# david-jk/BigGAN-Tensorflow

Measured on AMD Instinct MI355X. Metric: BigGAN-128 train-step images/sec, higher is better.
Workload: dtype bf16; 1 GPU; BigGAN-128 ch=96 bf16 (BASELINE config 3: global batch 256, 32/GPU over 8 GPUs); img_size=128, ch=96, per_gpu_batch=256, global_batch=256, da_policy=full, g_regularization=ortho_cosine, n_labels=0, gan_type=hinge, hip_graph=False, precision=bf16, parallelism=dp1

## Files before the change

### biggan-tensorflow_amd/csrc/elementwise.hip

```cpp
#include <stdlib.h>
#include <mutex>
#include "common.h"

namespace bg {

#define EW_BLOCK 256
#define EW_MAX_BLOCKS 2048

static inline int ew_grid(int64_t work_items) {
    int64_t b = (work_items + EW_BLOCK - 1) / EW_BLOCK;
    if (b > EW_MAX_BLOCKS) b = EW_MAX_BLOCKS;
    if (b < 1) b = 1;
    return (int)b;
}

__device__ __forceinline__ float4 ldg4(const float* p) { return *reinterpret_cast<const float4*>(p); }
__device__ __forceinline__ void stg4(float* p, const float4& v) { *reinterpret_cast<float4*>(p) = v; }

template <int NQ, int VEC, class Fn, class OutT>
__global__ __launch_bounds__(EW_BLOCK) void colreduce_kernel(Fn fn, OutT* out, float* part, int64_t qstride,
                                                             int64_t rows_per_seg, int C, int rows_per_block) {
    __shared__ float red[NQ * EW_BLOCK * VEC];
    const int CV = C / VEC;
    const int tx = CV < EW_BLOCK ? CV : EW_BLOCK;
    const int lanes = EW_BLOCK / tx;
    const int cq = threadIdx.x % tx, rl = threadIdx.x / tx;
    const int seg = blockIdx.y;
    const int64_t r0 = (int64_t)blockIdx.x * rows_per_block;
    int64_t r1 = r0 + rows_per_block;
    if (r1 > rows_per_seg) r1 = rows_per_seg;
    for (int cbase = 0; cbase < CV; cbase += tx) {
        const int cv = cbase + cq;
        float acc[NQ][VEC];
#pragma unroll
        for (int q = 0; q < NQ; ++q)
#pragma unroll
            for (int j = 0; j < VEC; ++j) acc[q][j] = 0.f;
        if (cv < CV && rl < lanes) {
            float acc4[4][NQ][VEC];
#pragma unroll
            for (int u = 0; u < 4; ++u)
#pragma unroll
                for (int q = 0; q < NQ; ++q)
#pragma unroll
                    for (int j = 0; j < VEC; ++j) acc4[u][q][j] = 0.f;
            int64_t r = r0 + rl;
            for (; r + 3 * (int64_t)lanes < r1; r += 4 * (int64_t)lanes) {
#pragma unroll
                for (int u = 0; u < 4; ++u) fn(seg, r + u * (int64_t)lanes, cv * VEC, acc4[u]);
            }
            for (; r < r1; r += lanes) fn(seg, r, cv * VEC, acc4[0]);
#pragma unroll
            for (int q = 0; q < NQ; ++q)
#pragma unroll
                for (int j = 0; j < VEC; ++j)
                    acc[q][j] = (acc4[0][q][j] + acc4[1][q][j]) + (acc4[2][q][j] + acc4[3][q][j]);
        }
#pragma unroll
        for (int q = 0; q < NQ; ++q)
#pragma unroll
            for (int j = 0; j < VEC; ++j) red[(q * VEC + j) * EW_BLOCK + threadIdx.x] = acc[q][j];
        __syncthreads();
        if (rl == 0 && cv < CV) {
#pragma unroll
            for (int q = 0; q < NQ; ++q)
#pragma unroll
                for (int j = 0; j < VEC; ++j) {
                    float s = 0.f;
                    for (int l = 0; l < lanes; ++l) s += red[(q * VEC + j) * EW_BLOCK + l * tx + cq];
// ... 81 lines not shown
        return nullptr;
    }
    if (ws[dev] && !captured[dev]) {
        (void)hipDeviceSynchronize();
        (void)hipFree(ws[dev]);
    }
    ws[dev] = p;
    cap[dev] = want;
    captured[dev] = false;
    return p;
}

static bool block_partials(int grid, int C, hipStream_t s, float** part) {
    *part = grid > 1 ? colreduce_workspace((size_t)grid * C, s) : nullptr;
    return grid <= 1 || *part;
}

static void finalize_block_partials(const float* part, float* out, int grid, int C, hipStream_t s) {
    if (part)
        hipLaunchKernelGGL((colreduce_finalize_kernel<1, float>), crf_grid(C), dim3(EW_BLOCK), 0, s, part, out,
                           (int64_t)0, 1, C, grid);
}

template <int NQ, bool WIDE = false, class Fn, class OutT>
static void launch_colreduce(Fn fn, OutT* out, int64_t qstride, int64_t rows_per_seg, int nseg, int C,
                             hipStream_t s) {
    static const int env_blocks = getenv("BG_COLRED_BLOCKS") ? atoi(getenv("BG_COLRED_BLOCKS")) : 0;
    const int64_t bytes = rows_per_seg * (int64_t)nseg * C * 4;
    const int target_blocks = env_blocks > 0 ? env_blocks : (bytes > (100ll << 20) ? 192 : 128);
    int64_t blocks_per_seg = (target_blocks + nseg - 1) / nseg;
    int64_t rpb = (rows_per_seg + blocks_per_seg - 1) / blocks_per_seg;
    if (rpb < 32) rpb = 32;
    blocks_per_seg = (rows_per_seg + rpb - 1) / rpb;
    float* part = nullptr;
    if (blocks_per_seg > 1) {
        part = colreduce_workspace((size_t)blocks_per_seg * nseg * NQ * C, s);
        if (!part) {
            g_ws_error = true;
            return;
        }
    }
    dim3 grid((unsigned)blocks_per_seg, (unsigned)nseg);
    bool launched = false;
    if constexpr (WIDE) {
        if (C % 8 == 0 && rows_per_seg * (int64_t)nseg * C >= (int64_t(16) << 20)) {
            hipLaunchKernelGGL((colreduce_kernel<NQ, 8, Fn, OutT>), grid, dim3(EW_BLOCK), 0, s, fn, out, part, qstride,
                               rows_per_seg, C, (int)rpb);
            launched = true;
        }
    }
    if (!launched) {
        if (C % 4 == 0)
            hipLaunchKernelGGL((colreduce_kernel<NQ, 4, Fn, OutT>), grid, dim3(EW_BLOCK), 0, s, fn, out, part, qstride,
                               rows_per_seg, C, (int)rpb);
        else
            hipLaunchKernelGGL((colreduce_kernel<NQ, 1, Fn, OutT>), grid, dim3(EW_BLOCK), 0, s, fn, out, part, qstride,
                               rows_per_seg, C, (int)rpb);
    }
    if (part) {
        const int64_t total = (int64_t)nseg * NQ * C;
        hipLaunchKernelGGL((colreduce_finalize_kernel<NQ, OutT>), crf_grid(total), dim3(EW_BLOCK), 0, s, part, out,
                           qstride, nseg, C, (int)blocks_per_seg);
    }
}

template <int VEC>
__device__ __forceinline__ void loadv(const float* p, float (&v)[VEC]) {
    if constexpr (VEC == 4) {
        float4 t = ldg4(p);
        v[0] = t.x;
        v[1] = t.y;
        v[2] = t.z;
        v[VEC - 1] = t.w;
    } else if constexpr (VEC == 8) {
        const float4 a = ldg4(p), b = ldg4(p + 4);
        v[0] = a.x; v[1] = a.y; v[2] = a.z; v[3] = a.w;
        v[4] = b.x; v[5] = b.y; v[6] = b.z; v[VEC - 1] = b.w;
    } else {
#pragma unroll
        for (int j = 0; j < VEC; ++j) v[j] = p[j];
    }
// ... 26 lines not shown
}
template <int VEC>
__device__ __forceinline__ void storev(float* p, const float (&v)[VEC]) {
    if constexpr (VEC == 4)
        stg4(p, make_float4(v[0], v[1], v[2], v[VEC - 1]));
    else {
#pragma unroll
        for (int j = 0; j < VEC; ++j) p[j] = v[j];
    }
}
template <int VEC>
__device__ __forceinline__ void storev(__bf16* p, const float (&v)[VEC]) {
    if constexpr (VEC == 4) {
        uint2 r;
        r.x = bf16_pack2(v[0], v[1]);
        r.y = bf16_pack2(v[2], v[VEC - 1]);
        *reinterpret_cast<uint2*>(p) = r;
    } else {
#pragma unroll
        for (int j = 0; j < VEC; ++j) p[j] = (__bf16)v[j];
    }
}

template <class TX>
struct BnStatsFnT {
    const TX* x;
    int C;
    template <int VEC>
    __device__ __forceinline__ void operator()(int, int64_t r, int c, float (&acc)[2][VEC]) const {
        float v[VEC];
        loadv<VEC>(x + r * C + c, v);
#pragma unroll
        for (int j = 0; j < VEC; ++j) {
            acc[0][j] += v[j];
            acc[1][j] += v[j] * v[j];
        }
    }
};

__global__ void bn_population_kernel(const float* __restrict__ pop_mean, const float* __restrict__ pop_var, float eps,
                                     float* __restrict__ mean, float* __restrict__ rstd, int C) {
    const int c = blockIdx.x * blockDim.x + threadIdx.x;
    if (c >= C) return;
    mean[c] = pop_mean[c];
    rstd[c] = rsqrtf(pop_var[c] + eps);
}

__global__ void bn_finalize_kernel(const double* sums, double count, float eps, float momentum, int unbiased,
                                   float* mean, float* rstd, float* mm, float* mv, int C) {
    const int c = blockIdx.x * blockDim.x + threadIdx.x;
// ... 165 lines not shown
    const float *mean, *rstd, *gamma, *beta, *alpha;
    int per_sample, HW, C;
    template <int VEC>
    __device__ __forceinline__ void operator()(int n, int64_t r, int c, float (&acc)[3][VEC]) const {
        const int64_t off = ((int64_t)n * HW + r) * C + c;
        float xv[VEC], dv[VEC], mu[VEC], rs[VEC], ga[VEC], be[VEC], al[VEC];
        loadv<VEC>(x + off, xv);
        loadv<VEC>(dy + off, dv);
        loadv<VEC>(mean + c, mu);
        loadv<VEC>(rstd + c, rs);
        loadv<VEC>(gamma + (per_sample ? (int64_t)n * C : 0) + c, ga);
        loadv<VEC>(beta + (per_sample ? (int64_t)n * C : 0) + c, be);
        if (alpha) loadv<VEC>(alpha + c, al);
#pragma unroll
        for (int j = 0; j < VEC; ++j) {
            const float xh = (xv[j] - mu[j]) * rs[j];
            const float pre = xh * ga[j] + be[j];
            const float g = alpha ? dv[j] * prelu_d(pre, al[j]) : dv[j];
            acc[0][j] += g;
            acc[1][j] += g * xh;
            acc[2][j] += alpha ? dv[j] * fminf(pre, 0.f) : 0.f;
        }
    }
};

template <int VEC, class TX, class TY>
__global__ __launch_bounds__(EW_BLOCK) void bn_apply_act_bwd_dx_t_kernel(
    const TX* __restrict__ x, const TY* __restrict__ dy, const float* __restrict__ mean,
    const float* __restrict__ rstd, const float* __restrict__ gamma, const float* __restrict__ beta, int per_sample,
    const float* __restrict__ alpha, const float* __restrict__ cm, TX* dx, const TX* add, int N, int HW, int C) {
    const int CV = C / VEC;
    const int64_t total = (int64_t)N * HW * CV;
    for (int64_t i = (int64_t)blockIdx.x * EW_BLOCK + threadIdx.x; i < total; i += (int64_t)gridDim.x * EW_BLOCK) {
        const int c = (int)(i % CV) * VEC;
        const int n = (int)(i / ((int64_t)HW * CV));
        float xv[VEC], dv[VEC], mu[VEC], rs[VEC], ga[VEC], be[VEC], al[VEC], m1[VEC], m2[VEC], out[VEC];
        loadv<VEC>(x + i * VEC, xv);
        loadv<VEC>(dy + i * VEC, dv);
        loadv<VEC>(mean + c, mu);
        loadv<VEC>(rstd + c, rs);
        loadv<VEC>(gamma + (per_sample ? (int64_t)n * C : 0) + c, ga);
        loadv<VEC>(beta + (per_sample ? (int64_t)n * C : 0) + c, be);
        loadv<VEC>(cm + c, m1);
        loadv<VEC>(cm + C + c, m2);
        if (alpha) loadv<VEC>(alpha + c, al);
#pragma unroll
// ... 49 lines not shown
                    dbeta[(int64_t)n * C + c] = a[u];
                    dgamma[(int64_t)n * C + c] = b[u];
                }
            }
        }
    }
    red[0][ry][cx] = s0; red[1][ry][cx] = s1; red[2][ry][cx] = s2; red[3][ry][cx] = g0; red[4][ry][cx] = g1;
    __syncthreads();
    if (ry != 0 || !live) return;
    s0 = (red[0][0][cx] + red[0][1][cx]) + (red[0][2][cx] + red[0][3][cx]);
    s1 = (red[1][0][cx] + red[1][1][cx]) + (red[1][2][cx] + red[1][3][cx]);
    s2 = (red[2][0][cx] + red[2][1][cx]) + (red[2][2][cx] + red[2][3][cx]);
    g0 = (red[3][0][cx] + red[3][1][cx]) + (red[3][2][cx] + red[3][3][cx]);
    g1 = (red[4][0][cx] + red[4][1][cx]) + (red[4][2][cx] + red[4][3][cx]);
    if (!per_sample) {
        dbeta[c] = (float)s0;
        dgamma[c] = (float)s1;
    }
    if (dalpha) dalpha[c] = (float)s2;
    cm[c] = (float)(g0 / count);
    cm[C + c] = (float)(g1 / count);
}

__device__ __forceinline__ void bf16x8_load(const __bf16* p, float (&v)[8]) {
    const uint4 r = *reinterpret_cast<const uint4*>(p);
    v[0] = __builtin_bit_cast(float, r.x << 16); v[1] = __builtin_bit_cast(float, r.x & 0xffff0000u);
    v[2] = __builtin_bit_cast(float, r.y << 16); v[3] = __builtin_bit_cast(float, r.y & 0xffff0000u);
    v[4] = __builtin_bit_cast(float, r.z << 16); v[5] = __builtin_bit_cast(float, r.z & 0xffff0000u);
    v[6] = __builtin_bit_cast(float, r.w << 16); v[7] = __builtin_bit_cast(float, r.w & 0xffff0000u);
}
__device__ __forceinline__ void bf16x8_store(__bf16* p, const float (&v)[8]) {
    uint4 r;
    r.x = bf16_pack2(v[0], v[1]); r.y = bf16_pack2(v[2], v[3]); r.z = bf16_pack2(v[4], v[5]); r.w = bf16_pack2(v[6], v[7]);
    *reinterpret_cast<uint4*>(p) = r;
}
__device__ __forceinline__ void f32x8_load(const float* p, float (&v)[8]) {
    const float4 a = ldg4(p), b = ldg4(p + 4);
    v[0] = a.x; v[1] = a.y; v[2] = a.z; v[3] = a.w; v[4] = b.x; v[5] = b.y; v[6] = b.z; v[7] = b.w;
}

__global__ __launch_bounds__(EW_BLOCK) void bn_apply_act_fwd_bf16x8_kernel(
    const __bf16* __restrict__ x, const float* __restrict__ mean, const float* __restrict__ rstd,
    const float* __restrict__ gamma, const float* __restrict__ beta, int per_sample, const float* __restrict__ alpha,
    __bf16* __restrict__ y, int rows, int HW, int CV) {
    const int gtid = blockIdx.x * EW_BLOCK + threadIdx.x;
    const int cv = gtid % CV, c = cv * 8, C = CV * 8;
    const int rstep = (gridDim.x * EW_BLOCK) / CV;
    float mu[8], rs[8], al[8], inv[8], sh[8];
    f32x8_load(mean + c, mu);
    f32x8_load(rstd + c, rs);
    if (alpha) f32x8_load(alpha + c, al);
    int r_end = 0;
    for (int r = gtid / CV; r < rows; r += rstep) {
        if (r >= r_end) {
            const int n = per_sample ? r / HW : 0;
            r_end = per_sample ? (n + 1) * HW : rows;
            float ga[8], be[8];
            f32x8_load(gamma + (int64_t)n * C * per_sample + c, ga);
            f32x8_load(beta + (int64_t)n * C * per_sample + c, be);
#pragma unroll
            for (int j = 0; j < 8; ++j) {
                inv[j] = rs[j] * ga[j];
                sh[j] = be[j] - mu[j] * inv[j];
            }
        }
        float xv[8], out[8];
        bf16x8_load(x + (int64_t)r * C + c, xv);
#pragma unroll
        for (int j = 0; j < 8; ++j) {
            const float v = xv[j] * inv[j] + sh[j];
            out[j] = alpha ? prelu_f(v, al[j]) : v;
        }
        bf16x8_store(y + (int64_t)r * C + c, out);
    }
}

__global__ __launch_bounds__(EW_BLOCK) void bn_apply_act_bwd_dx_bf16x8_kernel(
    const __bf16* __restrict__ x, const __bf16* __restrict__ dy, const float* __restrict__ mean,
    const float* __restrict__ rstd, const float* __restrict__ gamma, const float* __restrict__ beta, int per_sample,
    const float* __restrict__ alpha, const float* __restrict__ cm, __bf16* dx, const __bf16* add, int rows, int HW,
    int CV) {
    const int gtid = blockIdx.x * EW_BLOCK + threadIdx.x;
    const int cv = gtid % CV, c = cv * 8, C = CV * 8;
    const int rstep = (gridDim.x * EW_BLOCK) / CV;
    float mu[8], rs[8], al[8], m1[8], m2[8], ga[8], be[8];
    f32x8_load(mean + c, mu);
    f32x8_load(rstd + c, rs);
    f32x8_load(cm + c, m1);
    f32x8_load(cm + C + c, m2);
    if (alpha) f32x8_load(alpha + c, al);
    int r_end = 0;
    for (int r = gtid / CV; r < rows; r += rstep) {
        if (r >= r_end) {
            const int n = per_sample ? r / HW : 0;
            r_end = per_sample ? (n + 1) * HW : rows;
            f32x8_load(gamma + (int64_t)n * C * per_sample + c, ga);
            f32x8_load(beta + (int64_t)n * C * per_sample + c, be);
        }
        float xv[8], dv[8], out[8];
        bf16x8_load(x + (int64_t)r * C + c, xv);
        bf16x8_load(dy + (int64_t)r * C + c, dv);
#pragma unroll
        for (int j = 0; j < 8; ++j) {
            const float xh = (xv[j] - mu[j]) * rs[j];
            const float pre = xh * ga[j] + be[j];
            const float g = alpha ? dv[j] * prelu_d(pre, al[j]) : dv[j];
            out[j] = rs[j] * (g * ga[j] - m1[j] - xh * m2[j]);
        }
        if (add) {
            float av[8];
            bf16x8_load(add + (int64_t)r * C + c, av);
#pragma unroll
            for (int j = 0; j < 8; ++j) out[j] += av[j];
        }
        bf16x8_store(dx + (int64_t)r * C + c, out);
    }
}

template <bool BWD>
__global__ __launch_bounds__(EW_BLOCK) void prelu_bf16x8_kernel(const __bf16* __restrict__ x, const __bf16* __restrict__ dy,
                                                                 const float* __restrict__ alpha, __bf16* out,
                                                                 const __bf16* add, int rows, int CV) {
    const int gtid = blockIdx.x * EW_BLOCK + threadIdx.x;
    const int c = (gtid % CV) * 8, C = CV * 8;
    const int rstep = (gridDim.x * EW_BLOCK) / CV;
    float al[8];
    f32x8_load(alpha + c, al);
    for (int r = gtid / CV; r < rows; r += rstep) {
        float xv[8], dv[8], o[8];
        bf16x8_load(x + (int64_t)r * C + c, xv);
        if (BWD) bf16x8_load(dy + (int64_t)r * C + c, dv);
#pragma unroll
        for (int j = 0; j < 8; ++j) o[j] = BWD ? dv[j] * prelu_d(xv[j], al[j]) : prelu_f(xv[j], al[j]);
        if (BWD && add) {
            float av[8];
            bf16x8_load(add + (int64_t)r * C + c, av);
#pragma unroll
            for (int j = 0; j < 8; ++j) o[j] += av[j];
        }
        bf16x8_store(out + (int64_t)r * C + c, o);
    }
}

__global__ __launch_bounds__(EW_BLOCK) void lincomb_bf16x8_kernel(const __bf16* __restrict__ a, const float* sa_dev, float sa,
                                                                   const __bf16* __restrict__ b, float sb,
                                                                   __bf16* __restrict__ y, int64_t n8) {
    const float s = sa_dev ? *sa_dev : sa;
    for (int64_t i = (int64_t)blockIdx.x * EW_BLOCK + threadIdx.x; i < n8; i += (int64_t)gridDim.x * EW_BLOCK) {
        float av[8], bv[8], o[8];
        bf16x8_load(a + i * 8, av);
        if (b) {
            bf16x8_load(b + i * 8, bv);
#pragma unroll
            for (int j = 0; j < 8; ++j) o[j] = s * av[j] + sb * bv[j];
        } else {
#pragma unroll
            for (int j = 0; j < 8; ++j) o[j] = s * av[j];
        }
        bf16x8_store(y + i * 8, o);
    }
}

static inline int bn_x8_grid(int64_t rows, int CV) {
    int a = CV, b = EW_BLOCK;
    while (b) { const int t = a % b; a = b; b = t; }
    const int unit = CV / a;
    int64_t want = (rows * CV + EW_BLOCK - 1) / EW_BLOCK;
    if (want > 4096) want = 4096;
    if (want < 1) want = 1;
    return (int)((want + unit - 1) / unit * unit);
}

template <int VEC, class TX, class TY>
__global__ __launch_bounds__(EW_BLOCK) void prelu_fwd_t_kernel(const TX* __restrict__ x, const float* __restrict__ alpha,
                                                                TY* __restrict__ y, int64_t total_v, int C) {
    const int CV = C / VEC;
    for (int64_t i = (int64_t)blockIdx.x * EW_BLOCK + threadIdx.x; i < total_v; i += (int64_t)gridDim.x * EW_BLOCK) {
        const int c = (int)(i % CV) * VEC;
        float xv[VEC], al[VEC], out[VEC];
        loadv<VEC>(x + i * VEC, xv);
        loadv<VEC>(alpha + c, al);
#pragma unroll
        for (int j = 0; j < VEC; ++j) out[j] = prelu_f(xv[j], al[j]);
        storev<VEC>(y + i * VEC, out);
// ... 16 lines not shown
        if (add) {
            float av[VEC];
            loadv<VEC>(add + i * VEC, av);
#pragma unroll
            for (int j = 0; j < VEC; ++j) out[j] += av[j];
        }
        storev<VEC>(dx + i * VEC, out);
    }
}

template <class TX, class TY>
struct PreluDalphaFnT {
    const TX* x;
    const TY* dy;
    int C;
    template <int VEC>
    __device__ __forceinline__ void operator()(int, int64_t r, int c, float (&acc)[1][VEC]) const {
        float xv[VEC], dv[VEC];
        loadv<VEC>(x + r * C + c, xv);
        loadv<VEC>(dy + r * C + c, dv);
#pragma unroll
        for (int j = 0; j < VEC; ++j) acc[0][j] += dv[j] * fminf(xv[j], 0.f);
    }
};

template <class T>
struct BiasGradFnT {
    const T* dy;
    int C;
    template <int VEC>
    __device__ __forceinline__ void operator()(int, int64_t r, int c, float (&acc)[1][VEC]) const {
        float dv[VEC];
        loadv<VEC>(dy + r * C + c, dv);
#pragma unroll
        for (int j = 0; j < VEC; ++j) acc[0][j] += dv[j];
    }
};

__global__ __launch_bounds__(EW_BLOCK) void prelu_dalpha_thin_kernel(float* part, const float* __restrict__ x, const float* __restrict__ dy,
                                                                     float* __restrict__ dalpha, int64_t rows, int C) {
    __shared__ float red[4][EW_BLOCK];
    float acc[4] = {0.f, 0.f, 0.f, 0.f};
    const int64_t stride = (int64_t)gridDim.x * EW_BLOCK;
    int64_t r = (int64_t)blockIdx.x * EW_BLOCK + threadIdx.x;
    for (; r + 3 * stride < rows; r += 4 * stride) {
        float xv[4][4], gv[4][4];
#pragma unroll
        for (int u = 0; u < 4; ++u)
#pragma unroll
            for (int c = 0; c < 4; ++c)
                if (c < C) {
                    xv[u][c] = x[(r + u * stride) * C + c];
                    gv[u][c] = dy[(r + u * stride) * C + c];
                }
#pragma unroll
        for (int u = 0; u < 4; ++u)
// ... 1483 lines not shown
    const int tiles = taps * ((rows_per_tap + 63) / 64) * ((cols + 63) / 64);
    hipLaunchKernelGGL(weight_pack_kernel, dim3(tiles < 2048 ? tiles : 2048), dim3(EW_BLOCK), 0, as_stream(stream), w,
                       (__bf16*)pack_p, (__bf16*)pack_t, taps, rows_per_tap, cols);
    BG_LAUNCH_CHECK();
    return BG_OK;
}

int bg_bn_stats_t(const void* x, int x_dtype, double* sums, int64_t rows, int C, void* stream) {
    BG_REQUIRE(x && sums && rows > 0 && C > 0 && BG_DT_OK(x_dtype), "bg_bn_stats_t: bad argument");
    BG_DISPATCH_T(x_dtype, BnStatsFnT<T> fn{(const T*)x, C};
                  launch_colreduce<2, sizeof(T) == 2>(fn, sums, (int64_t)C, rows, 1, C, as_stream(stream)));
    BG_LAUNCH_CHECK();
    return BG_OK;
}

int bg_bn_apply_act_fwd_t(const void* x, int x_dtype, const float* mean, const float* rstd, const float* gamma,
                          const float* beta, int per_sample, const float* alpha, void* y, int y_dtype, int N, int HW,
                          int C, void* stream) {
    BG_REQUIRE(x && mean && rstd && gamma && beta && y && N > 0 && HW > 0 && C > 0 && BG_DT_OK(x_dtype) && BG_DT_OK(y_dtype),
               "bg_bn_apply_act_fwd_t: bad argument");
    const int64_t total = (int64_t)N * HW * C;
    if (x_dtype == BG_BF16 && y_dtype == BG_BF16 && C % 8 == 0 && (int64_t)N * HW < (int64_t(1) << 31) &&
        ((uintptr_t)x & 15) == 0 && ((uintptr_t)y & 15) == 0) {
        hipLaunchKernelGGL(bn_apply_act_fwd_bf16x8_kernel, dim3(bn_x8_grid((int64_t)N * HW, C / 8)), dim3(EW_BLOCK), 0,
                           as_stream(stream), (const __bf16*)x, mean, rstd, gamma, beta, per_sample, alpha, (__bf16*)y,
                           N * HW, HW, C / 8);
        BG_LAUNCH_CHECK();
        return BG_OK;
    }
    if (C % 4 == 0)
        BG_DISPATCH_XY(x_dtype, y_dtype,
                       hipLaunchKernelGGL((bn_apply_act_fwd_t_kernel<4, TX, TY>), dim3(ew_grid(total / 4)), dim3(EW_BLOCK),
                                          0, as_stream(stream), (const TX*)x, mean, rstd, gamma, beta, per_sample, alpha,
                                          (TY*)y, N, HW, C));
    else
        BG_DISPATCH_XY(x_dtype, y_dtype,
                       hipLaunchKernelGGL((bn_apply_act_fwd_t_kernel<1, TX, TY>), dim3(ew_grid(total)), dim3(EW_BLOCK), 0,
                                          as_stream(stream), (const TX*)x, mean, rstd, gamma, beta, per_sample, alpha,
                                          (TY*)y, N, HW, C));
    BG_LAUNCH_CHECK();
    return BG_OK;
}

int bg_bn_apply_act_bwd_reduce_t(const void* x, int x_dtype, const void* dy, int y_dtype, const float* mean,
                                 const float* rstd, const float* gamma, const float* beta, int per_sample,
                                 const float* alpha, float* part, int N, int HW, int C, void* stream) {
    BG_REQUIRE(x && dy && mean && rstd && gamma && beta && part && N > 0 && HW > 0 && C > 0 && BG_DT_OK(x_dtype) &&
                   BG_DT_OK(y_dtype), "bg_bn_apply_act_bwd_reduce_t: bad argument");
    if (zero_async(part, sizeof(float) * 3 * (size_t)N * C, as_stream(stream)) != hipSuccess) {
        set_error("bg_bn_apply_act_bwd_reduce_t: memset failed");
        return BG_ERR_LAUNCH;
    }
    BG_DISPATCH_XY(x_dtype, y_dtype,
                   BnBwdReduceFnT<TX, TY> fn{(const TX*)x, (const TY*)dy, mean, rstd, gamma, beta, alpha, per_sample, HW, C};
                   launch_colreduce<3, sizeof(TX) == 2 && sizeof(TY) == 2>(fn, part, (int64_t)N * C, HW, N, C,
                                                                           as_stream(stream)));
    BG_LAUNCH_CHECK();
    return BG_OK;
}

int bg_bn_apply_act_bwd_dx_t(const void* x, int x_dtype, const void* dy, int y_dtype, const float* mean, const float* rstd,
                             const float* gamma, const float* beta, int per_sample, const float* alpha, const float* cm,
                             void* dx, const void* dx_add, int N, int HW, int C, void* stream) {
    BG_REQUIRE(x && dy && mean && rstd && gamma && beta && cm && dx && N > 0 && HW > 0 && C > 0 && BG_DT_OK(x_dtype) &&
                   BG_DT_OK(y_dtype), "bg_bn_apply_act_bwd_dx_t: bad argument");
    const int64_t total = (int64_t)N * HW * C;
    if (x_dtype == BG_BF16 && y_dtype == BG_BF16 && C % 8 == 0 && (int64_t)N * HW < (int64_t(1) << 31) &&
        ((uintptr_t)x & 15) == 0 && ((uintptr_t)dy & 15) == 0 && ((uintptr_t)dx & 15) == 0 && ((uintptr_t)dx_add & 15) == 0) {
        hipLaunchKernelGGL(bn_apply_act_bwd_dx_bf16x8_kernel, dim3(bn_x8_grid((int64_t)N * HW, C / 8)), dim3(EW_BLOCK), 0,
                           as_stream(stream), (const __bf16*)x, (const __bf16*)dy, mean, rstd, gamma, beta, per_sample,
                           alpha, cm, (__bf16*)dx, (const __bf16*)dx_add, N * HW, HW, C / 8);
        BG_LAUNCH_CHECK();
        return BG_OK;
    }
    if (C % 4 == 0)
        BG_DISPATCH_XY(x_dtype, y_dtype,
                       hipLaunchKernelGGL((bn_apply_act_bwd_dx_t_kernel<4, TX, TY>), dim3(ew_grid(total / 4)),
                                          dim3(EW_BLOCK), 0, as_stream(stream), (const TX*)x, (const TY*)dy, mean, rstd,
                                          gamma, beta, per_sample, alpha, cm, (TX*)dx, (const TX*)dx_add, N, HW, C));
    else
        BG_DISPATCH_XY(x_dtype, y_dtype,
                       hipLaunchKernelGGL((bn_apply_act_bwd_dx_t_kernel<1, TX, TY>), dim3(ew_grid(total)), dim3(EW_BLOCK), 0,
                                          as_stream(stream), (const TX*)x, (const TY*)dy, mean, rstd, gamma, beta,
                                          per_sample, alpha, cm, (TX*)dx, (const TX*)dx_add, N, HW, C));
    BG_LAUNCH_CHECK();
    return BG_OK;
}

int bg_prelu_fwd_t(const void* x, int x_dtype, const float* alpha, void* y, int y_dtype, int64_t rows, int C,
                   void* stream) {
    BG_REQUIRE(x && alpha && y && rows > 0 && C > 0 && BG_DT_OK(x_dtype) && BG_DT_OK(y_dtype), "bg_prelu_fwd_t: bad argument");
    const int64_t total = rows * C;
    if (x_dtype == BG_BF16 && y_dtype == BG_BF16 && C % 8 == 0 && rows < (int64_t(1) << 31) && ((uintptr_t)x & 15) == 0 &&
        ((uintptr_t)y & 15) == 0) {
        hipLaunchKernelGGL((prelu_bf16x8_kernel<false>), dim3(bn_x8_grid(rows, C / 8)), dim3(EW_BLOCK), 0, as_stream(stream),
                           (const __bf16*)x, (const __bf16*)nullptr, alpha, (__bf16*)y, (const __bf16*)nullptr, (int)rows,
                           C / 8);
        BG_LAUNCH_CHECK();
        return BG_OK;
    }
    if (C % 4 == 0)
        BG_DISPATCH_XY(x_dtype, y_dtype,
                       hipLaunchKernelGGL((prelu_fwd_t_kernel<4, TX, TY>), dim3(ew_grid(total / 4)), dim3(EW_BLOCK), 0,
                                          as_stream(stream), (const TX*)x, alpha, (TY*)y, total / 4, C));
    else
        BG_DISPATCH_XY(x_dtype, y_dtype,
                       hipLaunchKernelGGL((prelu_fwd_t_kernel<1, TX, TY>), dim3(ew_grid(total)), dim3(EW_BLOCK), 0,
                                          as_stream(stream), (const TX*)x, alpha, (TY*)y, total, C));
    BG_LAUNCH_CHECK();
    return BG_OK;
}

int bg_prelu_bwd_t(const void* x, int x_dtype, const void* dy, int y_dtype, const float* alpha, void* dx, float* dalpha,
                   const void* dx_add, int64_t rows, int C, void* stream) {
    BG_REQUIRE(x && dy && alpha && rows > 0 && C > 0 && BG_DT_OK(x_dtype) && BG_DT_OK(y_dtype), "bg_prelu_bwd_t: bad argument");
    const int64_t total = rows * C;
    const bool x8 = x_dtype == BG_BF16 && y_dtype == BG_BF16 && C % 8 == 0 && rows < (int64_t(1) << 31) &&
                    ((uintptr_t)x & 15) == 0 && ((uintptr_t)dy & 15) == 0 && ((uintptr_t)dx & 15) == 0 &&
                    ((uintptr_t)dx_add & 15) == 0;
    if (dx && x8) {
        hipLaunchKernelGGL((prelu_bf16x8_kernel<true>), dim3(bn_x8_grid(rows, C / 8)), dim3(EW_BLOCK), 0, as_stream(stream),
                           (const __bf16*)x, (const __bf16*)dy, alpha, (__bf16*)dx, (const __bf16*)dx_add, (int)rows, C / 8);
        BG_LAUNCH_CHECK();
    } else if (dx) {
        if (C % 4 == 0)
            BG_DISPATCH_XY(x_dtype, y_dtype,
                           hipLaunchKernelGGL((prelu_bwd_dx_t_kernel<4, TX, TY>), dim3(ew_grid(total / 4)), dim3(EW_BLOCK),
                                              0, as_stream(stream), (const TX*)x, (const TY*)dy, alpha, (TX*)dx,
                                              (const TX*)dx_add, total / 4, C));
        else
            BG_DISPATCH_XY(x_dtype, y_dtype,
                           hipLaunchKernelGGL((prelu_bwd_dx_t_kernel<1, TX, TY>), dim3(ew_grid(total)), dim3(EW_BLOCK), 0,
                                              as_stream(stream), (const TX*)x, (const TY*)dy, alpha, (TX*)dx,
                                              (const TX*)dx_add, total, C));
        BG_LAUNCH_CHECK();
    }
    if (dalpha && x_dtype == BG_F32 && y_dtype == BG_F32 && C <= 4 && rows >= (int64_t(1) << 16)) {
        const int grid = 256;
        float* part = nullptr;
        if (!block_partials(grid, C, as_stream(stream), &part)) return BG_ERR_LAUNCH;
        hipLaunchKernelGGL(prelu_dalpha_thin_kernel, dim3(grid), dim3(EW_BLOCK), 0, as_stream(stream), part,
                           (const float*)x, (const float*)dy, dalpha, rows, C);
        finalize_block_partials(part, dalpha, grid, C, as_stream(stream));
        BG_LAUNCH_CHECK();
    } else if (dalpha) {
// ... 54 lines not shown
        BG_DISPATCH_T(x_dtype, hipLaunchKernelGGL((sum_pool_fwd_t_kernel<1, T>), dim3(ew_grid((int64_t)N * C)),
                                                  dim3(EW_BLOCK), 0, as_stream(stream), (const T*)x, y, N, HW, C));
    BG_LAUNCH_CHECK();
    return BG_OK;
}

int bg_sum_pool_bwd_t(const float* dy, void* dx, int x_dtype, int N, int HW, int C, void* stream) {
    BG_REQUIRE(dy && dx && N > 0 && HW > 0 && C > 0 && BG_DT_OK(x_dtype), "bg_sum_pool_bwd_t: bad argument");
    if (C % 4 == 0)
        BG_DISPATCH_T(x_dtype, hipLaunchKernelGGL((sum_pool_bwd_t_kernel<4, T>), dim3(ew_grid((int64_t)N * HW * C / 4)),
                                                  dim3(EW_BLOCK), 0, as_stream(stream), dy, (T*)dx, N, HW, C));
    else
        BG_DISPATCH_T(x_dtype, hipLaunchKernelGGL((sum_pool_bwd_t_kernel<1, T>), dim3(ew_grid((int64_t)N * HW * C)),
                                                  dim3(EW_BLOCK), 0, as_stream(stream), dy, (T*)dx, N, HW, C));
    BG_LAUNCH_CHECK();
    return BG_OK;
}

int bg_lincomb_t(const void* a, const float* sa_dev, float sa, const void* b, float sb, void* y, int dtype, int64_t n,
                 void* stream) {
    BG_REQUIRE(a && y && n > 0 && n % 4 == 0 && BG_DT_OK(dtype), "bg_lincomb_t: bad argument (n %% 4 == 0)");
    if (dtype == BG_BF16 && n % 8 == 0 && ((uintptr_t)a & 15) == 0 && ((uintptr_t)y & 15) == 0 &&
        (!b || ((uintptr_t)b & 15) == 0)) {
        hipLaunchKernelGGL(lincomb_bf16x8_kernel, dim3(ew_grid(n / 8)), dim3(EW_BLOCK), 0, as_stream(stream),
                           (const __bf16*)a, sa_dev, sa, (const __bf16*)b, sb, (__bf16*)y, n / 8);
        BG_LAUNCH_CHECK();
        return BG_OK;
    }
    BG_DISPATCH_T(dtype, hipLaunchKernelGGL((lincomb_t_kernel<T>), dim3(ew_grid(n / 4)), dim3(EW_BLOCK), 0, as_stream(stream),
                                            (const T*)a, sa_dev, sa, (const T*)b, sb, (T*)y, n / 4));
    BG_LAUNCH_CHECK();
    return BG_OK;
}

int bg_dot_t(const void* a, const void* b, int dtype, float* out_accum, int64_t n, void* stream) {
    BG_REQUIRE(a && b && out_accum && n > 0 && n % 4 == 0 && BG_DT_OK(dtype), "bg_dot_t: bad argument (n %% 4 == 0)");
    int rc = BG_OK;
    BG_DISPATCH_T(dtype, rc = launch_dot((const T*)a, (const T*)b, out_accum, n, as_stream(stream)));
    return rc;
}

int bg_bn_stats(const float* x, double* sums, int64_t rows, int C, void* stream) {
    return bg_bn_stats_t(x, BG_F32, sums, rows, C, stream);
}

int bg_bn_apply_act_fwd(const float* x, const float* mean, const float* rstd, const float* gamma, const float* beta,
                        int per_sample, const float* alpha, float* y, int N, int HW, int C, void* stream) {
    return bg_bn_apply_act_fwd_t(x, BG_F32, mean, rstd, gamma, beta, per_sample, alpha, y, BG_F32, N, HW, C, stream);
// ... 53 lines not shown
```

Before: 2865 images/sec.

## Batch loads ahead of math in column reductions and bf16x8 elementwise kernels

```diff
diff --git a/biggan-tensorflow_amd/csrc/elementwise.hip b/biggan-tensorflow_amd/csrc/elementwise.hip
--- a/biggan-tensorflow_amd/csrc/elementwise.hip
+++ b/biggan-tensorflow_amd/csrc/elementwise.hip
@@ -1,5 +1,6 @@
 #include <stdlib.h>
 #include <mutex>
+#include <type_traits>
 #include "common.h"
 
 namespace bg {
@@ -17,7 +18,7 @@
 __device__ __forceinline__ float4 ldg4(const float* p) { return *reinterpret_cast<const float4*>(p); }
 __device__ __forceinline__ void stg4(float* p, const float4& v) { *reinterpret_cast<float4*>(p) = v; }
 
-template <int NQ, int VEC, class Fn, class OutT>
+template <int NQ, int VEC, class Fn, class OutT, int K = 1>
 __global__ __launch_bounds__(EW_BLOCK) void colreduce_kernel(Fn fn, OutT* out, float* part, int64_t qstride,
                                                              int64_t rows_per_seg, int C, int rows_per_block) {
     __shared__ float red[NQ * EW_BLOCK * VEC];
@@ -45,6 +46,24 @@
 #pragma unroll
                     for (int j = 0; j < VEC; ++j) acc4[u][q][j] = 0.f;
             int64_t r = r0 + rl;
+            if constexpr (K > 1) {
+                const int64_t L = lanes;
+                typename Fn::template Ctx<VEC> cx;
+                fn.template ctx<VEC>(seg, cv * VEC, cx);
+                for (; r + (4 * K - 1) * L < r1; r += 4 * K * L) {
+                    typename Fn::template Raw<VEC> raw[K][4];
+#pragma unroll
+                    for (int k = 0; k < K; ++k)
+#pragma unroll
+                        for (int u = 0; u < 4; ++u)
+                            fn.template load<VEC>(seg, r + (4 * k + u) * L, cv * VEC, raw[k][u]);
+                    __builtin_amdgcn_sched_barrier(0);
+#pragma unroll
+                    for (int k = 0; k < K; ++k)
+#pragma unroll
+                        for (int u = 0; u < 4; ++u) fn.template accum<VEC>(cx, raw[k][u], acc4[u]);
+                }
+            }
             for (; r + 3 * (int64_t)lanes < r1; r += 4 * (int64_t)lanes) {
 #pragma unroll
                 for (int u = 0; u < 4; ++u) fn(seg, r + u * (int64_t)lanes, cv * VEC, acc4[u]);
@@ -172,10 +191,68 @@
                            (int64_t)0, 1, C, grid);
 }
 
+static inline int ew_pipe_env() {
+    const char* e = getenv("BG_EW_PIPE");
+    return e && *e ? atoi(e) : -1;
+}
+
+template <class Fn, class = void>
+struct ew_has_pipe : std::false_type {};
+template <class Fn>
+struct ew_has_pipe<Fn, std::void_t<typename Fn::pipelined>> : std::true_type {};
+
+template <int NQ, class Fn>
+static inline int colreduce_depth_rule(int64_t elements) {
+    if constexpr (ew_has_pipe<Fn>::value) {
+        const int e = ew_pipe_env();
+        if (e == 0) return 4;
+        if (e >= 8) return e >= 16 ? 16 : e >= 12 ? 12 : 8;
+        if (!Fn::bf16) return 4;
+        if (NQ == 3) return 8;
+        if (NQ == 2) return 12;
+        if (Fn::operands == 2) return elements >= (int64_t(64) << 20) ? 8 : 4;
+        return 16;
+    }
+    return 4;
+}
+
+template <int NQ, int VEC, class Fn, class OutT>
+static void colreduce_launch_depth(int depth, dim3 grid, hipStream_t s, Fn fn, OutT* out, float* part, int64_t qstride,
+                                   int64_t rows_per_seg, int C, int rpb) {
+    constexpr bool deep = !(NQ == 3 && VEC == 8);
+    if constexpr (ew_has_pipe<Fn>::value && !deep) {
+        if (depth >= 8) {
+            hipLaunchKernelGGL((colreduce_kernel<NQ, VEC, Fn, OutT, 2>), grid, dim3(EW_BLOCK), 0, s, fn, out, part, qstride,
+                               rows_per_seg, C, rpb);
+            return;
+        }
+    }
+    if constexpr (ew_has_pipe<Fn>::value && deep) {
+        if (depth == 8) {
+            hipLaunchKernelGGL((colreduce_kernel<NQ, VEC, Fn, OutT, 2>), grid, dim3(EW_BLOCK), 0, s, fn, out, part, qstride,
+                               rows_per_seg, C, rpb);
+            return;
+        }
+        if (depth == 12) {
+            hipLaunchKernelGGL((colreduce_kernel<NQ, VEC, Fn, OutT, 3>), grid, dim3(EW_BLOCK), 0, s, fn, out, part, qstride,
+                               rows_per_seg, C, rpb);
+            return;
+        }
+        if (depth == 16) {
+            hipLaunchKernelGGL((colreduce_kernel<NQ, VEC, Fn, OutT, 4>), grid, dim3(EW_BLOCK), 0, s, fn, out, part, qstride,
+                               rows_per_seg, C, rpb);
+            return;
+        }
+    }
+    hipLaunchKernelGGL((colreduce_kernel<NQ, VEC, Fn, OutT>), grid, dim3(EW_BLOCK), 0, s, fn, out, part, qstride,
+                       rows_per_seg, C, rpb);
+}
+
 template <int NQ, bool WIDE = false, class Fn, class OutT>
 static void launch_colreduce(Fn fn, OutT* out, int64_t qstride, int64_t rows_per_seg, int nseg, int C,
                              hipStream_t s) {
-    static const int env_blocks = getenv("BG_COLRED_BLOCKS") ? atoi(getenv("BG_COLRED_BLOCKS")) : 0;
+    const char* eb = getenv("BG_COLRED_BLOCKS");
+    const int env_blocks = eb ? atoi(eb) : 0;
     const int64_t bytes = rows_per_seg * (int64_t)nseg * C * 4;
     const int target_blocks = env_blocks > 0 ? env_blocks : (bytes > (100ll << 20) ? 192 : 128);
     int64_t blocks_per_seg = (target_blocks + nseg - 1) / nseg;
@@ -191,22 +268,19 @@
         }
     }
     dim3 grid((unsigned)blocks_per_seg, (unsigned)nseg);
-    bool launched = false;
+    const int depth = colreduce_depth_rule<NQ, Fn>(rows_per_seg * (int64_t)nseg * C);
+    bool wide = false;
     if constexpr (WIDE) {
-        if (C % 8 == 0 && rows_per_seg * (int64_t)nseg * C >= (int64_t(16) << 20)) {
-            hipLaunchKernelGGL((colreduce_kernel<NQ, 8, Fn, OutT>), grid, dim3(EW_BLOCK), 0, s, fn, out, part, qstride,
-                               rows_per_seg, C, (int)rpb);
-            launched = true;
-        }
-    }
-    if (!launched) {
-        if (C % 4 == 0)
-            hipLaunchKernelGGL((colreduce_kernel<NQ, 4, Fn, OutT>), grid, dim3(EW_BLOCK), 0, s, fn, out, part, qstride,
-                               rows_per_seg, C, (int)rpb);
-        else
-            hipLaunchKernelGGL((colreduce_kernel<NQ, 1, Fn, OutT>), grid, dim3(EW_BLOCK), 0, s, fn, out, part, qstride,
-                               rows_per_seg, C, (int)rpb);
-    }
+        wide = C % 8 == 0 && rows_per_seg * (int64_t)nseg * C >= (int64_t(16) << 20);
+        if (wide) colreduce_launch_depth<NQ, 8>(depth, grid, s, fn, out, part, qstride, rows_per_seg, C, (int)rpb);
+    }
+    if (wide)
+        ;
+    else if (C % 4 == 0)
+        colreduce_launch_depth<NQ, 4>(depth, grid, s, fn, out, part, qstride, rows_per_seg, C, (int)rpb);
+    else
+        hipLaunchKernelGGL((colreduce_kernel<NQ, 1, Fn, OutT>), grid, dim3(EW_BLOCK), 0, s, fn, out, part, qstride,
+                           rows_per_seg, C, (int)rpb);
     if (part) {
         const int64_t total = (int64_t)nseg * NQ * C;
         hipLaunchKernelGGL((colreduce_finalize_kernel<NQ, OutT>), crf_grid(total), dim3(EW_BLOCK), 0, s, part, out,
@@ -279,10 +353,75 @@
     }
 }
 
+struct NoCtx {};
+template <class T, int VEC>
+struct RawVec;
+typedef uint32_t ew_u32x4 __attribute__((ext_vector_type(4)));
+typedef uint32_t ew_u32x2 __attribute__((ext_vector_type(2)));
+typedef float ew_f32x4 __attribute__((ext_vector_type(4)));
+template <int VEC>
+struct RawVec<float, VEC> {
+    static_assert(VEC == 4 || VEC == 8, "RawVec<float>: 16- or 32-byte vectors");
+    ew_f32x4 r[VEC / 4];
+    __device__ __forceinline__ void load(const float* p) {
+#pragma unroll
+        for (int h = 0; h < VEC / 4; ++h) r[h] = *reinterpret_cast<const ew_f32x4*>(p + 4 * h);
+    }
+    __device__ __forceinline__ void get(float (&o)[VEC]) const {
+#pragma unroll
+        for (int j = 0; j < VEC; ++j) o[j] = r[j / 4][j % 4];
+    }
+};
+template <>
+struct RawVec<__bf16, 8> {
+    ew_u32x4 r;
+    __device__ __forceinline__ void load(const __bf16* p) { r = *reinterpret_cast<const ew_u32x4*>(p); }
+    __device__ __forceinline__ void get(float (&o)[8]) const {
+#pragma unroll
+        for (int j = 0; j < 4; ++j) {
+            o[2 * j] = __builtin_bit_cast(float, r[j] << 16);
+            o[2 * j + 1] = __builtin_bit_cast(float, r[j] & 0xffff0000u);
+        }
+    }
+};
+template <>
+struct RawVec<__bf16, 4> {
+    ew_u32x2 r;
+    __device__ __forceinline__ void load(const __bf16* p) { r = *reinterpret_cast<const ew_u32x2*>(p); }
+    __device__ __forceinline__ void get(float (&o)[4]) const {
+#pragma unroll
+        for (int j = 0; j < 2; ++j) {
+            o[2 * j] = __builtin_bit_cast(float, r[j] << 16);
+            o[2 * j + 1] = __builtin_bit_cast(float, r[j] & 0xffff0000u);
+        }
+    }
+};
+
 template <class TX>
 struct BnStatsFnT {
     const TX* x;
     int C;
+    using pipelined = void;
+    static constexpr int operands = 1;
+    static constexpr bool bf16 = sizeof(TX) == 2;
+    template <int VEC>
+    using Raw = RawVec<TX, VEC>;
+    template <int VEC>
+    using Ctx = NoCtx;
+    template <int VEC>
+    __device__ __forceinline__ void ctx(int, int, NoCtx&) const {}
+    template <int VEC>
+    __device__ __forceinline__ void load(int, int64_t r, int c, Raw<VEC>& w) const { w.load(x + r * C + c); }
+    template <int VEC>
+    __device__ __forceinline__ void accum(const NoCtx&, const Raw<VEC>& w, float (&acc)[2][VEC]) const {
+        float v[VEC];
+        w.get(v);
+#pragma unroll
+        for (int j = 0; j < VEC; ++j) {
+            acc[0][j] += v[j];
+            acc[1][j] += v[j] * v[j];
+        }
+    }
     template <int VEC>
     __device__ __forceinline__ void operator()(int, int64_t r, int c, float (&acc)[2][VEC]) const {
         float v[VEC];
@@ -494,6 +633,48 @@
             acc[2][j] += alpha ? dv[j] * fminf(pre, 0.f) : 0.f;
         }
     }
+    using pipelined = void;
+    static constexpr int operands = 2;
+    static constexpr bool bf16 = sizeof(TX) == 2 && sizeof(TY) == 2;
+    template <int VEC>
+    struct Raw {
+        RawVec<TX, VEC> x;
+        RawVec<TY, VEC> dy;
+    };
+    template <int VEC>
+    __device__ __forceinline__ void load(int n, int64_t r, int c, Raw<VEC>& w) const {
+        const int64_t off = ((int64_t)n * HW + r) * C + c;
+        w.x.load(x + off);
+        w.dy.load(dy + off);
+    }
+    template <int VEC>
+    struct Ctx {
+        float mu[VEC], rs[VEC], ga[VEC], be[VEC], al[VEC];
+    };
+    template <int VEC>
+    __device__ __forceinline__ void ctx(int n, int c, Ctx<VEC>& k) const {
+        loadv<VEC>(mean + c, k.mu);
+        loadv<VEC>(rstd + c, k.rs);
+        loadv<VEC>(gamma + (per_sample ? (int64_t)n * C : 0) + c, k.ga);
+        loadv<VEC>(beta + (per_sample ? (int64_t)n * C : 0) + c, k.be);
+        if (alpha) loadv<VEC>(alpha + c, k.al);
+    }
+    template <int VEC>
+    __device__ __forceinline__ void accum(const Ctx<VEC>& k, const Raw<VEC>& w, float (&acc)[3][VEC]) const {
+        float xv[VEC], dv[VEC];
+        w.x.get(xv);
+        w.dy.get(dv);
+        const float (&mu)[VEC] = k.mu, (&rs)[VEC] = k.rs, (&ga)[VEC] = k.ga, (&be)[VEC] = k.be, (&al)[VEC] = k.al;
+#pragma unroll
+        for (int j = 0; j < VEC; ++j) {
+            const float xh = (xv[j] - mu[j]) * rs[j];
+            const float pre = xh * ga[j] + be[j];
+            const float g = alpha ? dv[j] * prelu_d(pre, al[j]) : dv[j];
+            acc[0][j] += g;
+            acc[1][j] += g * xh;
+            acc[2][j] += alpha ? dv[j] * fminf(pre, 0.f) : 0.f;
+        }
+    }
 };
 
 template <int VEC, class TX, class TY>
@@ -589,6 +770,13 @@
     cm[C + c] = (float)(g1 / count);
 }
 
+__device__ __forceinline__ uint4 bf16x8_raw(const __bf16* p) { return *reinterpret_cast<const uint4*>(p); }
+__device__ __forceinline__ void bf16x8_widen(const uint4& r, float (&v)[8]) {
+    v[0] = __builtin_bit_cast(float, r.x << 16); v[1] = __builtin_bit_cast(float, r.x & 0xffff0000u);
+    v[2] = __builtin_bit_cast(float, r.y << 16); v[3] = __builtin_bit_cast(float, r.y & 0xffff0000u);
+    v[4] = __builtin_bit_cast(float, r.z << 16); v[5] = __builtin_bit_cast(float, r.z & 0xffff0000u);
+    v[6] = __builtin_bit_cast(float, r.w << 16); v[7] = __builtin_bit_cast(float, r.w & 0xffff0000u);
+}
 __device__ __forceinline__ void bf16x8_load(const __bf16* p, float (&v)[8]) {
     const uint4 r = *reinterpret_cast<const uint4*>(p);
     v[0] = __builtin_bit_cast(float, r.x << 16); v[1] = __builtin_bit_cast(float, r.x & 0xffff0000u);
@@ -606,6 +794,7 @@
     v[0] = a.x; v[1] = a.y; v[2] = a.z; v[3] = a.w; v[4] = b.x; v[5] = b.y; v[6] = b.z; v[7] = b.w;
 }
 
+template <int U>
 __global__ __launch_bounds__(EW_BLOCK) void bn_apply_act_fwd_bf16x8_kernel(
     const __bf16* __restrict__ x, const float* __restrict__ mean, const float* __restrict__ rstd,
     const float* __restrict__ gamma, const float* __restrict__ beta, int per_sample, const float* __restrict__ alpha,
@@ -618,7 +807,39 @@
     f32x8_load(rstd + c, rs);
     if (alpha) f32x8_load(alpha + c, al);
     int r_end = 0;
-    for (int r = gtid / CV; r < rows; r += rstep) {
+    int r = gtid / CV;
+    if constexpr (U > 1) {
+        for (; (int64_t)r + (int64_t)(U - 1) * rstep < rows; r += U * rstep) {
+            uint4 xr[U];
+#pragma unroll
+            for (int u = 0; u < U; ++u) xr[u] = bf16x8_raw(x + (int64_t)(r + u * rstep) * C + c);
+#pragma unroll
+            for (int u = 0; u < U; ++u) {
+                const int ru = r + u * rstep;
+                if (ru >= r_end) {
+                    const int n = per_sample ? ru / HW : 0;
+                    r_end = per_sample ? (n + 1) * HW : rows;
+                    float ga[8], be[8];
+                    f32x8_load(gamma + (int64_t)n * C * per_sample + c, ga);
+                    f32x8_load(beta + (int64_t)n * C * per_sample + c, be);
+#pragma unroll
+                    for (int j = 0; j < 8; ++j) {
+                        inv[j] = rs[j] * ga[j];
+                        sh[j] = be[j] - mu[j] * inv[j];
+                    }
+                }
+                float xv[8], out[8];
+                bf16x8_widen(xr[u], xv);
+#pragma unroll
+                for (int j = 0; j < 8; ++j) {
+                    const float v = xv[j] * inv[j] + sh[j];
+                    out[j] = alpha ? prelu_f(v, al[j]) : v;
+                }
+                bf16x8_store(y + (int64_t)ru * C + c, out);
+            }
+        }
+    }
+    for (; r < rows; r += rstep) {
         if (r >= r_end) {
             const int n = per_sample ? r / HW : 0;
             r_end = per_sample ? (n + 1) * HW : rows;
@@ -642,6 +863,7 @@
     }
 }
 
+template <int U>
 __global__ __launch_bounds__(EW_BLOCK) void bn_apply_act_bwd_dx_bf16x8_kernel(
     const __bf16* __restrict__ x, const __bf16* __restrict__ dy, const float* __restrict__ mean,
     const float* __restrict__ rstd, const float* __restrict__ gamma, const float* __restrict__ beta, int per_sample,
@@ -657,7 +879,47 @@
     f32x8_load(cm + C + c, m2);
     if (alpha) f32x8_load(alpha + c, al);
     int r_end = 0;
-    for (int r = gtid / CV; r < rows; r += rstep) {
+    int r = gtid / CV;
+    if constexpr (U > 1) {
+        for (; (int64_t)r + (int64_t)(U - 1) * rstep < rows; r += U * rstep) {
+            uint4 xr[U], dr[U], ar[U];
+#pragma unroll
+            for (int u = 0; u < U; ++u) {
+                const int64_t off = (int64_t)(r + u * rstep) * C + c;
+                xr[u] = bf16x8_raw(x + off);
+                dr[u] = bf16x8_raw(dy + off);
+                if (add) ar[u] = bf16x8_raw(add + off);
+            }
+#pragma unroll
+            for (int u = 0; u < U; ++u) {
+                const int ru = r + u * rstep;
+                if (ru >= r_end) {
+                    const int n = per_sample ? ru / HW : 0;
+                    r_end = per_sample ? (n + 1) * HW : rows;
+                    f32x8_load(gamma + (int64_t)n * C * per_sample + c, ga);
+                    f32x8_load(beta + (int64_t)n * C * per_sample + c, be);
+                }
+                float xv[8], dv[8], out[8];
+                bf16x8_widen(xr[u], xv);
+                bf16x8_widen(dr[u], dv);
+#pragma unroll
+                for (int j = 0; j < 8; ++j) {
+                    const float xh = (xv[j] - mu[j]) * rs[j];
+                    const float pre = xh * ga[j] + be[j];
+                    const float g = alpha ? dv[j] * prelu_d(pre, al[j]) : dv[j];
+                    out[j] = rs[j] * (g * ga[j] - m1[j] - xh * m2[j]);
+                }
+                if (add) {
+                    float av[8];
+                    bf16x8_widen(ar[u], av);
+#pragma unroll
+                    for (int j = 0; j < 8; ++j) out[j] += av[j];
+                }
+                bf16x8_store(dx + (int64_t)ru * C + c, out);
+            }
+        }
+    }
+    for (; r < rows; r += rstep) {
         if (r >= r_end) {
             const int n = per_sample ? r / HW : 0;
             r_end = per_sample ? (n + 1) * HW : rows;
@@ -684,7 +946,7 @@
     }
 }
 
-template <bool BWD>
+template <bool BWD, int U>
 __global__ __launch_bounds__(EW_BLOCK) void prelu_bf16x8_kernel(const __bf16* __restrict__ x, const __bf16* __restrict__ dy,
                                                                  const float* __restrict__ alpha, __bf16* out,
                                                                  const __bf16* add, int rows, int CV) {
@@ -693,7 +955,35 @@
     const int rstep = (gridDim.x * EW_BLOCK) / CV;
     float al[8];
     f32x8_load(alpha + c, al);
-    for (int r = gtid / CV; r < rows; r += rstep) {
+    int r = gtid / CV;
+    if constexpr (U > 1) {
+        for (; (int64_t)r + (int64_t)(U - 1) * rstep < rows; r += U * rstep) {
+            uint4 xr[U], dr[U], ar[U];
+#pragma unroll
+            for (int u = 0; u < U; ++u) {
+                const int64_t off = (int64_t)(r + u * rstep) * C + c;
+                xr[u] = bf16x8_raw(x + off);
+                if (BWD) dr[u] = bf16x8_raw(dy + off);
+                if (BWD && add) ar[u] = bf16x8_raw(add + off);
+            }
+#pragma unroll
+            for (int u = 0; u < U; ++u) {
+                float xv[8], dv[8], o[8];
+                bf16x8_widen(xr[u], xv);
+                if (BWD) bf16x8_widen(dr[u], dv);
+#pragma unroll
+                for (int j = 0; j < 8; ++j) o[j] = BWD ? dv[j] * prelu_d(xv[j], al[j]) : prelu_f(xv[j], al[j]);
+                if (BWD && add) {
+                    float av[8];
+                    bf16x8_widen(ar[u], av);
+#pragma unroll
+                    for (int j = 0; j < 8; ++j) o[j] += av[j];
+                }
+                bf16x8_store(out + (int64_t)(r + u * rstep) * C + c, o);
+            }
+        }
+    }
+    for (; r < rows; r += rstep) {
         float xv[8], dv[8], o[8];
         bf16x8_load(x + (int64_t)r * C + c, xv);
         if (BWD) bf16x8_load(dy + (int64_t)r * C + c, dv);
@@ -709,11 +999,38 @@
     }
 }
 
+template <int U>
 __global__ __launch_bounds__(EW_BLOCK) void lincomb_bf16x8_kernel(const __bf16* __restrict__ a, const float* sa_dev, float sa,
                                                                    const __bf16* __restrict__ b, float sb,
                                                                    __bf16* __restrict__ y, int64_t n8) {
     const float s = sa_dev ? *sa_dev : sa;
-    for (int64_t i = (int64_t)blockIdx.x * EW_BLOCK + threadIdx.x; i < n8; i += (int64_t)gridDim.x * EW_BLOCK) {
+    const int64_t step = (int64_t)gridDim.x * EW_BLOCK;
+    int64_t i = (int64_t)blockIdx.x * EW_BLOCK + threadIdx.x;
+    if constexpr (U > 1) {
+        for (; i + (U - 1) * step < n8; i += U * step) {
+            uint4 ar[U], br[U];
+#pragma unroll
+            for (int u = 0; u < U; ++u) {
+                ar[u] = bf16x8_raw(a + (i + u * step) * 8);
+                if (b) br[u] = bf16x8_raw(b + (i + u * step) * 8);
+            }
+#pragma unroll
+            for (int u = 0; u < U; ++u) {
+                float av[8], bv[8], o[8];
+                bf16x8_widen(ar[u], av);
+                if (b) {
+                    bf16x8_widen(br[u], bv);
+#pragma unroll
+                    for (int j = 0; j < 8; ++j) o[j] = s * av[j] + sb * bv[j];
+                } else {
+#pragma unroll
+                    for (int j = 0; j < 8; ++j) o[j] = s * av[j];
+                }
+                bf16x8_store(y + (i + u * step) * 8, o);
+            }
+        }
+    }
+    for (; i < n8; i += step) {
         float av[8], bv[8], o[8];
         bf16x8_load(a + i * 8, av);
         if (b) {
@@ -727,6 +1044,30 @@
         bf16x8_store(y + i * 8, o);
     }
 }
+
+#define X8_RULE_BN_FWD 1
+#define X8_RULE_BN_BWD 1
+#define X8_RULE_PRELU_FWD 1
+#define X8_RULE_PRELU_BWD 1
+#define X8_RULE_LINCOMB 1
+static inline int x8_rows_rule(int rule) {
+    const int e = ew_pipe_env();
+    return e < 0 ? rule : e >= 4 ? 4 : e >= 2 ? 2 : 1;
+}
+#define EW_DISPATCH_U(u, ...)                                                                                          \
+    do {                                                                                                               \
+        const int u_ = (u);                                                                                            \
+        if (u_ == 4) {                                                                                                 \
+            constexpr int U = 4;                                                                                       \
+            __VA_ARGS__;                                                                                               \
+        } else if (u_ == 2) {                                                                                          \
+            constexpr int U = 2;                                                                                       \
+            __VA_ARGS__;                                                                                               \
+        } else {                                                                                                       \
+            constexpr int U = 1;                                                                                       \
+            __VA_ARGS__;                                                                                               \
+        }                                                                                                              \
+    } while (0)
 
 static inline int bn_x8_grid(int64_t rows, int CV) {
     int a = CV, b = EW_BLOCK;
@@ -789,6 +1130,31 @@
 #pragma unroll
         for (int j = 0; j < VEC; ++j) acc[0][j] += dv[j] * fminf(xv[j], 0.f);
     }
+    using pipelined = void;
+    static constexpr int operands = 2;
+    static constexpr bool bf16 = sizeof(TX) == 2 && sizeof(TY) == 2;
+    template <int VEC>
+    struct Raw {
+        RawVec<TX, VEC> x;
+        RawVec<TY, VEC> dy;
+    };
+    template <int VEC>
+    using Ctx = NoCtx;
+    template <int VEC>
+    __device__ __forceinline__ void ctx(int, int, NoCtx&) const {}
+    template <int VEC>
+    __device__ __forceinline__ void load(int, int64_t r, int c, Raw<VEC>& w) const {
+        w.x.load(x + r * C + c);
+        w.dy.load(dy + r * C + c);
+    }
+    template <int VEC>
+    __device__ __forceinline__ void accum(const NoCtx&, const Raw<VEC>& w, float (&acc)[1][VEC]) const {
+        float xv[VEC], dv[VEC];
+        w.x.get(xv);
+        w.dy.get(dv);
+#pragma unroll
+        for (int j = 0; j < VEC; ++j) acc[0][j] += dv[j] * fminf(xv[j], 0.f);
+    }
 };
 
 template <class T>
@@ -799,6 +1165,24 @@
     __device__ __forceinline__ void operator()(int, int64_t r, int c, float (&acc)[1][VEC]) const {
         float dv[VEC];
         loadv<VEC>(dy + r * C + c, dv);
+#pragma unroll
+        for (int j = 0; j < VEC; ++j) acc[0][j] += dv[j];
+    }
+    using pipelined = void;
+    static constexpr int operands = 1;
+    static constexpr bool bf16 = sizeof(T) == 2;
+    template <int VEC>
+    using Raw = RawVec<T, VEC>;
+    template <int VEC>
+    using Ctx = NoCtx;
+    template <int VEC>
+    __device__ __forceinline__ void ctx(int, int, NoCtx&) const {}
+    template <int VEC>
+    __device__ __forceinline__ void load(int, int64_t r, int c, Raw<VEC>& w) const { w.load(dy + r * C + c); }
+    template <int VEC>
+    __device__ __forceinline__ void accum(const NoCtx&, const Raw<VEC>& w, float (&acc)[1][VEC]) const {
+        float dv[VEC];
+        w.get(dv);
 #pragma unroll
         for (int j = 0; j < VEC; ++j) acc[0][j] += dv[j];
     }
@@ -2328,9 +2712,10 @@
     const int64_t total = (int64_t)N * HW * C;
     if (x_dtype == BG_BF16 && y_dtype == BG_BF16 && C % 8 == 0 && (int64_t)N * HW < (int64_t(1) << 31) &&
         ((uintptr_t)x & 15) == 0 && ((uintptr_t)y & 15) == 0) {
-        hipLaunchKernelGGL(bn_apply_act_fwd_bf16x8_kernel, dim3(bn_x8_grid((int64_t)N * HW, C / 8)), dim3(EW_BLOCK), 0,
-                           as_stream(stream), (const __bf16*)x, mean, rstd, gamma, beta, per_sample, alpha, (__bf16*)y,
-                           N * HW, HW, C / 8);
+        EW_DISPATCH_U(x8_rows_rule(X8_RULE_BN_FWD),
+                      hipLaunchKernelGGL(bn_apply_act_fwd_bf16x8_kernel<U>, dim3(bn_x8_grid((int64_t)N * HW, C / 8)),
+                                         dim3(EW_BLOCK), 0, as_stream(stream), (const __bf16*)x, mean, rstd, gamma, beta,
+                                         per_sample, alpha, (__bf16*)y, N * HW, HW, C / 8));
         BG_LAUNCH_CHECK();
         return BG_OK;
     }
@@ -2373,9 +2758,11 @@
     const int64_t total = (int64_t)N * HW * C;
     if (x_dtype == BG_BF16 && y_dtype == BG_BF16 && C % 8 == 0 && (int64_t)N * HW < (int64_t(1) << 31) &&
         ((uintptr_t)x & 15) == 0 && ((uintptr_t)dy & 15) == 0 && ((uintptr_t)dx & 15) == 0 && ((uintptr_t)dx_add & 15) == 0) {
-        hipLaunchKernelGGL(bn_apply_act_bwd_dx_bf16x8_kernel, dim3(bn_x8_grid((int64_t)N * HW, C / 8)), dim3(EW_BLOCK), 0,
-                           as_stream(stream), (const __bf16*)x, (const __bf16*)dy, mean, rstd, gamma, beta, per_sample,
-                           alpha, cm, (__bf16*)dx, (const __bf16*)dx_add, N * HW, HW, C / 8);
+        EW_DISPATCH_U(x8_rows_rule(X8_RULE_BN_BWD),
+                      hipLaunchKernelGGL(bn_apply_act_bwd_dx_bf16x8_kernel<U>, dim3(bn_x8_grid((int64_t)N * HW, C / 8)),
+                                         dim3(EW_BLOCK), 0, as_stream(stream), (const __bf16*)x, (const __bf16*)dy, mean,
+                                         rstd, gamma, beta, per_sample, alpha, cm, (__bf16*)dx, (const __bf16*)dx_add,
+                                         N * HW, HW, C / 8));
         BG_LAUNCH_CHECK();
         return BG_OK;
     }
@@ -2399,9 +2786,10 @@
     const int64_t total = rows * C;
     if (x_dtype == BG_BF16 && y_dtype == BG_BF16 && C % 8 == 0 && rows < (int64_t(1) << 31) && ((uintptr_t)x & 15) == 0 &&
         ((uintptr_t)y & 15) == 0) {
-        hipLaunchKernelGGL((prelu_bf16x8_kernel<false>), dim3(bn_x8_grid(rows, C / 8)), dim3(EW_BLOCK), 0, as_stream(stream),
-                           (const __bf16*)x, (const __bf16*)nullptr, alpha, (__bf16*)y, (const __bf16*)nullptr, (int)rows,
-                           C / 8);
+        EW_DISPATCH_U(x8_rows_rule(X8_RULE_PRELU_FWD),
+                      hipLaunchKernelGGL((prelu_bf16x8_kernel<false, U>), dim3(bn_x8_grid(rows, C / 8)), dim3(EW_BLOCK), 0,
+                                         as_stream(stream), (const __bf16*)x, (const __bf16*)nullptr, alpha, (__bf16*)y,
+                                         (const __bf16*)nullptr, (int)rows, C / 8));
         BG_LAUNCH_CHECK();
         return BG_OK;
     }
@@ -2425,8 +2813,10 @@
                     ((uintptr_t)x & 15) == 0 && ((uintptr_t)dy & 15) == 0 && ((uintptr_t)dx & 15) == 0 &&
                     ((uintptr_t)dx_add & 15) == 0;
     if (dx && x8) {
-        hipLaunchKernelGGL((prelu_bf16x8_kernel<true>), dim3(bn_x8_grid(rows, C / 8)), dim3(EW_BLOCK), 0, as_stream(stream),
-                           (const __bf16*)x, (const __bf16*)dy, alpha, (__bf16*)dx, (const __bf16*)dx_add, (int)rows, C / 8);
+        EW_DISPATCH_U(x8_rows_rule(X8_RULE_PRELU_BWD),
+                      hipLaunchKernelGGL((prelu_bf16x8_kernel<true, U>), dim3(bn_x8_grid(rows, C / 8)), dim3(EW_BLOCK), 0,
+                                         as_stream(stream), (const __bf16*)x, (const __bf16*)dy, alpha, (__bf16*)dx,
+                                         (const __bf16*)dx_add, (int)rows, C / 8));
         BG_LAUNCH_CHECK();
     } else if (dx) {
         if (C % 4 == 0)
@@ -2527,8 +2917,10 @@
     BG_REQUIRE(a && y && n > 0 && n % 4 == 0 && BG_DT_OK(dtype), "bg_lincomb_t: bad argument (n %% 4 == 0)");
     if (dtype == BG_BF16 && n % 8 == 0 && ((uintptr_t)a & 15) == 0 && ((uintptr_t)y & 15) == 0 &&
         (!b || ((uintptr_t)b & 15) == 0)) {
-        hipLaunchKernelGGL(lincomb_bf16x8_kernel, dim3(ew_grid(n / 8)), dim3(EW_BLOCK), 0, as_stream(stream),
-                           (const __bf16*)a, sa_dev, sa, (const __bf16*)b, sb, (__bf16*)y, n / 8);
+        EW_DISPATCH_U(x8_rows_rule(X8_RULE_LINCOMB),
+                      hipLaunchKernelGGL(lincomb_bf16x8_kernel<U>, dim3(ew_grid(n / 8)), dim3(EW_BLOCK), 0,
+                                         as_stream(stream), (const __bf16*)a, sa_dev, sa, (const __bf16*)b, sb,
+                                         (__bf16*)y, n / 8));
         BG_LAUNCH_CHECK();
         return BG_OK;
     }
```

After: 2876 images/sec, median of 6. Within noise of the previous version (+0.4%).
